# DRL-Navigation/DDRL4NAV

Hardware: AMD Instinct MI355X
Metric: env-steps/sec (whole node) + PPO update ms, Pong 256 envs at 1/2/4/8 GPUs (higher is better)
Workload: dtype f32 (f16x3 MFMA planes, fp32 accumulate)

## Files before the change

ddrl4nav_amd/csrc/fc2.hip:

```cpp
#include "engine2.h"

namespace ddrl {



struct FcFwdB {
  static constexpr int PITCH = 80, PLANE = 128 * PITCH, B_OFF = NPL * PLANE, LDS_BYTES = 2 * NPL * PLANE;
};

template <bool SPLIT>
__global__ __launch_bounds__(256) void fc_fwd_planes_kernel(const float* __restrict__ a3, int64_t a3_es, const unsigned short* __restrict__ wlb,
                                                            const float* __restrict__ amax, const float* __restrict__ params, int64_t bias_off0,
                                                            int64_t bias_off1, float* __restrict__ h, int64_t h_es, int n, int ne, int nsplit,
                                                            float* __restrict__ part, const float* __restrict__ smax, int smax_es) {
  using K = FcFwdB;
  extern __shared__ __attribute__((aligned(16))) char ldsf[];
  const int tid = threadIdx.x, lane = tid & 63, wave = tid >> 6, l31 = lane & 31, hi = lane >> 5;
  const int wr = wave >> 1, wc = wave & 1;
  int bx = blockIdx.x, by = blockIdx.y, bz = blockIdx.z;
  if (!SPLIT && (gridDim.y & 7) == 0) {
    const int lin = bx + 4 * by, xcd = lin & 7, q = lin >> 3;
    bx = q & 3, by = (q >> 2) * 8 + xcd;
  }
  if (SPLIT) {
    const int G = 4 * (int)gridDim.y, nz = (int)gridDim.z, lin = bx + 4 * by + G * bz, full = (nz & ~7) * G;
    int g, m;
    if (lin < full) {
      const int xcd = lin & 7, r = lin >> 3;
      g = (r / G) * 8 + xcd, m = r % G;
    } else {
      const int l2 = lin - full, xcd = l2 & 7, rest = nz & 7;
      if (rest == 4) {
        g = (nz & ~7) + (xcd >> 1), m = (l2 >> 3) * 2 + (xcd & 1);
      } else {
        g = (nz & ~7) + l2 / G, m = l2 % G;
      }
    }
    bz = g, bx = m & 3, by = m >> 2;
  }
  const int e = SPLIT ? bz % ne : bz, split = SPLIT ? bz / ne : 0, n0 = bx * 128, b0 = by * 128;
  float sa = plane_scale(amax[amax_idx(AMAX_A3, e)]), inv = 1.0f / (sa * plane_scale(amax[amax_idx(AMAX_WL, e)]));
  const int k4 = tid & 7, rr = tid >> 3;
  const float* asrc[4];
#pragma unroll
  for (int j = 0; j < 4; ++j) asrc[j] = a3 + e * a3_es + (int64_t)min(b0 + rr + 32 * j, n - 1) * FLAT + k4 * 4;
  const int k8 = tid & 3, cc = tid >> 2;
  const unsigned short* wsrc = wlb + (int64_t)e * 3 * FLAT * FEAT + (int64_t)(n0 + cc) * FLAT + k8 * 8;
  int aA[2], bB[2];
#pragma unroll
  for (int i = 0; i < 2; ++i) aA[i] = (wr * 64 + i * 32 + l31) * K::PITCH + hi * 16;
#pragma unroll
  for (int j = 0; j < 2; ++j) bB[j] = K::B_OFF + (wc * 64 + j * 32 + l31) * K::PITCH + hi * 16;
  constexpr int DEPTH = SPLIT ? 4 : 1;
  f4 ar[DEPTH][4], wrg[DEPTH][2][NPL];
  auto fetch = [&](int kb, int slot) {
#pragma unroll
    for (int j = 0; j < 4; ++j) ar[slot][j] = ld4(asrc[j] + kb * 32);
#pragma unroll
    for (int j = 0; j < 2; ++j)
#pragma unroll
      for (int p = 0; p < NPL; ++p) wrg[slot][j][p] = *(const f4*)(wsrc + (int64_t)p * FLAT * FEAT + (int64_t)j * 64 * FLAT + kb * 32);
  };
  auto commit = [&](int slot) {
#pragma unroll
    for (int j = 0; j < 4; ++j) {
      const f4 v = ar[slot][j];
      unsigned pa[NPL], pb[NPL];
      split_planes_c(v.x, v.y, sa, pa);
      split_planes_c(v.z, v.w, sa, pb);
      char* d = ldsf + (rr + 32 * j) * K::PITCH + k4 * 8;
#pragma unroll
      for (int p = 0; p < NPL; ++p) *(uint2*)(d + p * K::PLANE) = make_uint2(pa[p], pb[p]);
    }
#pragma unroll
    for (int j = 0; j < 2; ++j)
#pragma unroll
      for (int p = 0; p < NPL; ++p) *(f4*)(ldsf + K::B_OFF + p * K::PLANE + (cc + 64 * j) * K::PITCH + k8 * 16) = wrg[slot][j][p];
  };
  f32x16 acc[2][2];
#pragma unroll
  for (int i = 0; i < 2; ++i)
#pragma unroll
    for (int j = 0; j < 2; ++j)
#pragma unroll
      for (int r = 0; r < 16; ++r) acc[i][j][r] = 0.0f;
  auto compute = [&]() {
#pragma unroll
    for (int kg = 0; kg < 2; ++kg) {
      frag8 a[NPL][2], b[NPL][2];
#pragma unroll
      for (int p = 0; p < NPL; ++p) {
#pragma unroll
        for (int i = 0; i < 2; ++i) a[p][i] = *(const frag8*)(ldsf + aA[i] + p * K::PLANE + kg * 32);
#pragma unroll
        for (int j = 0; j < 2; ++j) b[p][j] = *(const frag8*)(ldsf + bB[j] + p * K::PLANE + kg * 32);
      }
#pragma unroll
      for (int t = 0; t < NPROD; ++t)
#pragma unroll
        for (int i = 0; i < 2; ++i)
#pragma unroll
          for (int j = 0; j < 2; ++j) acc[i][j] = mfma_planes(a[PA[t]][i], b[PB[t]][j], acc[i][j]);
    }
  };
  if constexpr (SPLIT) {
    constexpr int PER = (FLAT / 32) / FC_ACT_SPLITS;
    const int kb0 = split * PER;
#pragma unroll
    for (int d = 0; d < DEPTH && d < PER; ++d) fetch(kb0 + d, d);
    if (smax != nullptr) {
      float m = 0.0f;
      for (int i = tid; i < n; i += 256) m = fmaxf(m, smax[e * smax_es + i]);
      m = wave_fmax(m);
      float* red = (float*)ldsf;
      if (lane == 0) red[wave] = m;
      __syncthreads();
      const float a3top = fmaxf(fmaxf(red[0], red[1]), fmaxf(red[2], red[3]));
      __syncthreads();
      sa = plane_scale(a3top), inv = 1.0f / (sa * plane_scale(amax[amax_idx(AMAX_WL, e)]));
    }
    commit(0);
    if (DEPTH < PER) fetch(kb0 + DEPTH, 0);
    __syncthreads();
#pragma unroll
    for (int k = 0; k < PER; ++k) {
      compute();
      __syncthreads();
      if (k + 1 < PER) {
        commit((k + 1) % DEPTH);
        if (k + 1 + DEPTH < PER) fetch(kb0 + k + 1 + DEPTH, (k + 1) % DEPTH);
      }
      __syncthreads();
    }
  } else {
    constexpr int NKB = FLAT / 32;
    fetch(0, 0);
    commit(0);
    fetch(1, 0);
    __syncthreads();
    for (int kb = 0; kb < NKB; ++kb) {
      compute();
      __syncthreads();
      if (kb + 1 < NKB) {
        commit(0);
        if (kb + 2 < NKB) fetch(kb + 2, 0);
      }
      __syncthreads();
    }
  }
#pragma unroll
  for (int j = 0; j < 2; ++j) {
    const int nn = n0 + wc * 64 + j * 32 + l31;
    const float bias = SPLIT ? 0.0f : params[(e ? bias_off1 : bias_off0) + nn];
    float* dst = SPLIT ? part + ((int64_t)split * 2 + e) * n * FEAT : h + e * h_es;
#pragma unroll
    for (int i = 0; i < 2; ++i)
#pragma unroll
      for (int r = 0; r < 16; ++r) {
        const int b = b0 + wr * 64 + i * 32 + acc_row(r, hi);
        if (b < n) dst[(int64_t)b * FEAT + nn] = acc[i][j][r] * inv + bias;
      }
  }
}

void launch_fc_forward2(const EncCall& c, bool allow_split, hipStream_t st, bool per_sample_max) {
  const Workspace& w = *c.ws;
  const int64_t MB = c.max_batch;
  const int nsplit = allow_split ? fc_forward_splits(c.n) : 1;
  ProfRange pr(c.prof, nsplit > 1 ? "FcFwdSplit" : "FcFwd", st);
  {
    lds_limit_once<fc_fwd_planes_kernel<false>>((int)FcFwdB::LDS_BYTES);
    lds_limit_once<fc_fwd_planes_kernel<true>>((int)FcFwdB::LDS_BYTES);
    const dim3 grid(FEAT / 128, (c.n + 127) / 128, c.L->NE * nsplit);
    if (nsplit > 1)
      hipLaunchKernelGGL(fc_fwd_planes_kernel<true>, grid, dim3(256), FcFwdB::LDS_BYTES, st, w.a3, MB * FLAT, w.wlb, w.amax, c.params,
                         c.L->enc_base[0] + c.L->enc.lb, c.L->enc_base[c.L->NE - 1] + c.L->enc.lb, w.h, MB * FEAT, c.n, c.L->NE, nsplit, w.wpart,
                         per_sample_max ? w.actmax : (const float*)nullptr, ACT_FUSED_MAX);
    else
      hipLaunchKernelGGL(fc_fwd_planes_kernel<false>, grid, dim3(256), FcFwdB::LDS_BYTES, st, w.a3, MB * FLAT, w.wlb, w.amax, c.params,
                         c.L->enc_base[0] + c.L->enc.lb, c.L->enc_base[c.L->NE - 1] + c.L->enc.lb, w.h, MB * FEAT, c.n, c.L->NE, 1, w.wpart,
                         (const float*)nullptr, 0);
  }
}

struct FcDgradB {
  static constexpr int KBK = 32, WPE = 2, PITCH = 2 * KBK + 16, PLANE = 128 * PITCH, B_OFF = NPL * PLANE, LDS_BYTES = 2 * NPL * PLANE;
  static constexpr int NAQ = KBK / 4, ARJ = 128 * NAQ / 256, AROWS = 256 / NAQ;
  static constexpr int NWF = KBK / 8, WJ = 128 * NWF / 256, WCOLS = 256 / NWF;
};
__global__ __launch_bounds__(256) __attribute__((amdgpu_waves_per_eu(FcDgradB::WPE, FcDgradB::WPE))) void fc_dgrad_planes_kernel(const float* __restrict__ dh, int64_t dh_es, const unsigned short* __restrict__ wdlb,
                                                              float* __restrict__ amax, const unsigned* __restrict__ m3, float* __restrict__ dz3, int64_t a3_es, int n) {
  using K = FcDgradB;
  extern __shared__ __attribute__((aligned(16))) char ldsg[];
  const int tid = threadIdx.x, lane = tid & 63, wave = tid >> 6, l31 = lane & 31, hi = lane >> 5;
  const int wr = wave >> 1, wc = wave & 1;
  int bx = blockIdx.x, by = blockIdx.y;
  if ((gridDim.y & 7) == 0) {
    const int lin = bx + 25 * by, xcd = lin & 7, q = lin >> 3;
    if ((gridDim.y & 63) != 0) {
      bx = q % 25, by = (q / 25) * 8 + xcd;
    } else {
      const int blk = q / 40, r = q % 40;
      bx = (blk % 5) * 5 + r % 5, by = ((blk / 5) * 8 + r / 5) * 8 + xcd;
    }
  }
  const int e = blockIdx.z, k0 = bx * 128, b0 = by * 128;
  const float sa = plane_scale(amax[amax_idx(AMAX_DH, e)]), inv = 1.0f / (sa * plane_scale(amax[amax_idx(AMAX_WL, e)]));
  const int n4 = tid % K::NAQ, rr = tid / K::NAQ;
  const float* asrc[K::ARJ];
#pragma unroll
  for (int j = 0; j < K::ARJ; ++j) asrc[j] = dh + e * dh_es + (int64_t)min(b0 + rr + K::AROWS * j, n - 1) * FEAT + n4 * 4;
  const int n8 = tid % K::NWF, cc = tid / K::NWF;
  const unsigned short* wsrc[K::WJ];
#pragma unroll
  for (int j = 0; j < K::WJ; ++j) wsrc[j] = wdlb + (int64_t)e * 3 * FLAT * FEAT + (int64_t)min(k0 + cc + K::WCOLS * j, FLAT - 1) * FEAT + n8 * 8;
  int aA[2], bB[2];
#pragma unroll
  for (int i = 0; i < 2; ++i) aA[i] = (wr * 64 + i * 32 + l31) * K::PITCH + hi * 16;
#pragma unroll
  for (int j = 0; j < 2; ++j) bB[j] = K::B_OFF + (wc * 64 + j * 32 + l31) * K::PITCH + hi * 16;
  f4 ar[K::ARJ], wrg[K::WJ][NPL];
  auto fetch = [&](int kb) {
#pragma unroll
    for (int j = 0; j < K::ARJ; ++j) ar[j] = ld4(asrc[j] + kb * K::KBK);
#pragma unroll
    for (int j = 0; j < K::WJ; ++j)
#pragma unroll
      for (int p = 0; p < NPL; ++p) wrg[j][p] = *(const f4*)(wsrc[j] + (int64_t)p * FLAT * FEAT + kb * K::KBK);
  };
  auto commit = [&]() {
#pragma unroll
    for (int j = 0; j < K::ARJ; ++j) {
      const f4 v = ar[j];
      unsigned pa[NPL], pb[NPL];
      split_planes_c(v.x, v.y, sa, pa);
      split_planes_c(v.z, v.w, sa, pb);
      char* d = ldsg + (rr + K::AROWS * j) * K::PITCH + n4 * 8;
#pragma unroll
      for (int p = 0; p < NPL; ++p) *(uint2*)(d + p * K::PLANE) = make_uint2(pa[p], pb[p]);
    }
#pragma unroll
    for (int j = 0; j < K::WJ; ++j)
#pragma unroll
      for (int p = 0; p < NPL; ++p) *(f4*)(ldsg + K::B_OFF + p * K::PLANE + (cc + K::WCOLS * j) * K::PITCH + n8 * 16) = wrg[j][p];
  };
  f32x16 acc[2][2];
#pragma unroll
  for (int i = 0; i < 2; ++i)
#pragma unroll
    for (int j = 0; j < 2; ++j)
#pragma unroll
      for (int r = 0; r < 16; ++r) acc[i][j][r] = 0.0f;
  constexpr int NKB = FEAT / K::KBK;
  fetch(0);
  commit();
  fetch(1);
  __syncthreads();
  for (int kb = 0; kb < NKB; ++kb) {
#pragma unroll
    for (int kg = 0; kg < K::KBK / 16; ++kg) {
      frag8 a[NPL][2], b[NPL][2];
#pragma unroll
      for (int p = 0; p < NPL; ++p) {
#pragma unroll
        for (int i = 0; i < 2; ++i) a[p][i] = *(const frag8*)(ldsg + aA[i] + p * K::PLANE + kg * 32);
#pragma unroll
        for (int j = 0; j < 2; ++j) b[p][j] = *(const frag8*)(ldsg + bB[j] + p * K::PLANE + kg * 32);
      }
#pragma unroll
      for (int t = 0; t < NPROD; ++t)
#pragma unroll
        for (int i = 0; i < 2; ++i)
#pragma unroll
          for (int j = 0; j < 2; ++j) acc[i][j] = mfma_planes(a[PA[t]][i], b[PB[t]][j], acc[i][j]);
    }
    __syncthreads();
    if (kb + 1 < NKB) {
      commit();
      if (kb + 2 < NKB) fetch(kb + 2);
    }
    __syncthreads();
  }
  float big = 0.0f;
#pragma unroll
  for (int j = 0; j < 2; ++j) {
    const int k = k0 + wc * 64 + j * 32 + l31;
    if (k >= FLAT) continue;
    const int ch = k / 49, pix = k % 49;
    const int mbit = 16 * (ch >> 5) + 15 - ((ch & 3) + 4 * ((ch & 31) >> 3));
    const unsigned* mp = m3 + (int64_t)e * (a3_es / FLAT) * 98 + pix * 2 + ((ch >> 2) & 1);
#pragma unroll
    for (int i = 0; i < 2; ++i) {
      unsigned mw[16];
#pragma unroll
      for (int r = 0; r < 16; ++r) {
        const int b = min(b0 + wr * 64 + i * 32 + acc_row(r, hi), n - 1);
        mw[r] = mp[(int64_t)b * 98];
      }
#pragma unroll
      for (int r = 0; r < 16; ++r) {
        const int b = b0 + wr * 64 + i * 32 + acc_row(r, hi);
        const float g = leaky_bit(mw[r], mbit, acc[i][j][r] * inv);
        if (b < n) {
          dz3[e * a3_es + (int64_t)b * FLAT + k] = g;
          big = fmaxf(big, fabsf(g));
        }
      }
    }
  }
  amax_update(big, amax + amax_idx(AMAX_DZ3, e));
}

struct FcWgradB {
  static constexpr int KB = 32, PITCH = 320, PLANE = KB * PITCH, B_OFF = NPL * PLANE, LDS_BYTES = 2 * NPL * PLANE;
  static constexpr int64_t SLAB = (int64_t)FEAT * FLAT + FEAT;
};

__global__ __launch_bounds__(256) void fc_wgrad_planes_kernel(const float* __restrict__ dh, int64_t dh_es, const float* __restrict__ a3,
                                                              int64_t a3_es, const float* __restrict__ amax, const float* __restrict__ gsc,
                                                              int64_t gsc_es, float* __restrict__ part, int n, int nsplit, int ne) {
  using K = FcWgradB;
  extern __shared__ __attribute__((aligned(16))) char ldsw[];
  const int tid = threadIdx.x, lane = tid & 63, wave = tid >> 6, l31 = lane & 31, hi = lane >> 5;
  const int wr = wave >> 1, wc = wave & 1;
  const int unit = (int)(blockIdx.x >> 5) * 8 + (int)(blockIdx.x & 7);
  if (unit >= 25 * ne * nsplit) return;
  const int bx = unit % 25, by = (int)(blockIdx.x >> 3) & 3, bz = unit / 25;
  const int e = bz % ne, split = bz / ne;
  const float sd = WGRAD_HEADROOM * plane_scale(amax[amax_idx(AMAX_DH, e)]) / amax[amax_idx(AMAX_GMAX, e)], sa = plane_scale(amax[amax_idx(AMAX_A3, e)]),
              inv = 1.0f / (sd * sa);
  const float* gs = gsc + e * gsc_es;
  const int k0 = bx * 128, n0 = by * 128;
  const int nkb = (n + K::KB - 1) / K::KB;
  const int per = (nkb + nsplit - 1) / nsplit;
  const int kb_begin = split * per, kb_end = min(nkb, kb_begin + per);
  const int c4 = tid & 31, kk = tid >> 5;
  const float* dsrc = dh + e * dh_es + n0 + c4 * 4;
  const float* asrc = a3 + e * a3_es + min(k0 + c4 * 4, FLAT - 4);
  const int g16 = lane >> 4, q = (lane >> 2) & 3, pp = lane & 3;
  int aA[2], bB[2];
#pragma unroll
  for (int i = 0; i < 2; ++i) aA[i] = (8 * (g16 >> 1) + q) * K::PITCH + (wr * 64 + i * 32 + 16 * (g16 & 1) + 4 * pp) * 2;
#pragma unroll
  for (int j = 0; j < 2; ++j) bB[j] = K::B_OFF + (8 * (g16 >> 1) + q) * K::PITCH + (wc * 64 + j * 32 + 16 * (g16 & 1) + 4 * pp) * 2;
  f4 dr[4], ar[4];
  float gr[4];
  f4 bsum = zero4();
  const bool bias_owner = (bx == 0);
  auto fetch = [&](int kb) {
#pragma unroll
    for (int j = 0; j < 4; ++j) {
      const int64_t row = min(kb * K::KB + kk + 8 * j, n - 1);
      dr[j] = ld4(dsrc + row * FEAT);
      ar[j] = ld4(asrc + row * FLAT);
      gr[j] = gs[row];
    }
  };
  auto commit = [&](int kb) {
    if (kb * K::KB + K::KB > n) {
      rare_path();
#pragma unroll
      for (int j = 0; j < 4; ++j)
        if (kb * K::KB + kk + 8 * j >= n) dr[j] = zero4();
      rare_path();
    }
#pragma unroll
    for (int j = 0; j < 4; ++j) {
      char* d = ldsw + (kk + 8 * j) * K::PITCH + c4 * 8;
      unsigned pa[NPL], pb[NPL];
      const float sdj = sd * gr[j];
      split_planes(dr[j].x, dr[j].y, sdj, pa);
      split_planes(dr[j].z, dr[j].w, sdj, pb);
#pragma unroll
      for (int p = 0; p < NPL; ++p) *(uint2*)(d + p * K::PLANE) = make_uint2(pa[p], pb[p]);
      split_planes(ar[j].x, ar[j].y, sa, pa);
      split_planes(ar[j].z, ar[j].w, sa, pb);
#pragma unroll
      for (int p = 0; p < NPL; ++p) *(uint2*)(d + K::B_OFF + p * K::PLANE) = make_uint2(pa[p], pb[p]);
    }
    if (bias_owner) bsum += (dr[0] * gr[0] + dr[1] * gr[1]) + (dr[2] * gr[2] + dr[3] * gr[3]);
  };
  f32x16 acc[2][2];
#pragma unroll
  for (int i = 0; i < 2; ++i)
#pragma unroll
    for (int j = 0; j < 2; ++j)
#pragma unroll
      for (int r = 0; r < 16; ++r) acc[i][j][r] = 0.0f;
  if (kb_begin < kb_end) {
    fetch(kb_begin);
    commit(kb_begin);
    if (kb_begin + 1 < kb_end) fetch(kb_begin + 1);
    __syncthreads();
    for (int kb = kb_begin; kb < kb_end; ++kb) {
#pragma unroll
      for (int kg = 0; kg < 2; ++kg) {
        frag8 a[NPL][2], b[NPL][2];
#pragma unroll
        for (int p = 0; p < NPL; ++p) {
          const int off = p * K::PLANE + kg * 16 * K::PITCH;
#pragma unroll
          for (int i = 0; i < 2; ++i) a[p][i] = tr_frag(ldsw, aA[i] + off, aA[i] + off + 4 * K::PITCH);
#pragma unroll
          for (int j = 0; j < 2; ++j) b[p][j] = tr_frag(ldsw, bB[j] + off, bB[j] + off + 4 * K::PITCH);
        }
#pragma unroll
        for (int t = 0; t < NPROD; ++t)
#pragma unroll
          for (int i = 0; i < 2; ++i)
#pragma unroll
            for (int j = 0; j < 2; ++j) acc[i][j] = mfma_planes(a[PA[t]][i], b[PB[t]][j], acc[i][j]);
      }
      __syncthreads();
      if (kb + 1 < kb_end) {
        commit(kb + 1);
        if (kb + 2 < kb_end) fetch(kb + 2);
      }
      __syncthreads();
    }
  }
  float* slab = part + ((int64_t)split * 2 + e) * K::SLAB;
#pragma unroll
  for (int j = 0; j < 2; ++j) {
    const int k = k0 + wc * 64 + j * 32 + l31;
    if (k >= FLAT) continue;
#pragma unroll
    for (int i = 0; i < 2; ++i)
#pragma unroll
      for (int r = 0; r < 16; ++r) slab[(int64_t)(n0 + wr * 64 + i * 32 + acc_row(r, hi)) * FLAT + k] = acc[i][j][r] * inv;
  }
  if (bias_owner) {
    float* red = (float*)ldsw;
    st4(red + kk * 128 + c4 * 4, bsum);
    __syncthreads();
    if (tid < 128) {
      float s = 0.0f;
#pragma unroll
      for (int t = 0; t < 8; ++t) s += red[t * 128 + tid];
      slab[(int64_t)FEAT * FLAT + n0 + tid] = s;
    }
  }
}

void launch_fc_backward2(const EncCall& c, float* grads, hipStream_t st, int part) {
  const Workspace& w = *c.ws;
  const int64_t MB = c.max_batch;
  const ParamLayout& L = *c.L;
  const int S = c.splits->fc;
  if (part != 1) {
    {
      ProfRange pr(c.prof, "FcWgrad", st);
      lds_limit_once<fc_wgrad_planes_kernel>((int)FcWgradB::LDS_BYTES);
      const dim3 wgrid((unsigned)((25 * L.NE * S + 7) / 8 * 32));
      hipLaunchKernelGGL(fc_wgrad_planes_kernel, wgrid, dim3(256), FcWgradB::LDS_BYTES, st, w.dh, MB * FEAT, w.a3, MB * FLAT, w.amax, w.gsc, MB,
                         w.wpart, c.n, S, L.NE);
    }
    ProfRange pr(c.prof, "reduce_partials", st);
    launch_reduce_partials(w.wpart, S, FcWgradB::SLAB, L.NE, grads, L.enc_base[0] + L.enc.lw, L.enc_base[1] + L.enc.lw, st);
  }
  if (part != 2) {
    ProfRange pr(c.prof, "FcDgrad", st);
    lds_limit_once<fc_dgrad_planes_kernel>((int)FcDgradB::LDS_BYTES);
    hipLaunchKernelGGL(fc_dgrad_planes_kernel, dim3((FLAT + 127) / 128, (c.n + 127) / 128, L.NE), dim3(256), FcDgradB::LDS_BYTES, st, w.dh, MB * FEAT,
                       w.wdlb, w.amax, w.m3, w.dz3, MB * FLAT, c.n);
  }
}

}
```

Measured before the change: 262,200.

## Retile FC dgrad kernel to 128x224 tiles with exact column coverage

Reshapes the FC data-gradient GEMM tile from 128x128 (2x2 waves, each 64x64) to 128 rows by 224 columns, where each wave owns 32 rows and all 7 column fragments. Since 224 divides FLAT (3136) exactly, the padded, clamped last column tile and its wasted MFMA work go away, and each wave reuses its A fragment across 7 B fragments. The XCD block swizzle is reworked for 14 column tiles. In exchange, LDS and accumulator register use per block grow and the grid has fewer blocks, which may reduce occupancy or cause spills at WPE=2.

```diff
diff --git a/ddrl4nav_amd/csrc/fc2.hip b/ddrl4nav_amd/csrc/fc2.hip
--- a/ddrl4nav_amd/csrc/fc2.hip
+++ b/ddrl4nav_amd/csrc/fc2.hip
@@ -184,49 +184,47 @@
 }
 
 struct FcDgradB {
-  static constexpr int KBK = 32, WPE = 2, PITCH = 2 * KBK + 16, PLANE = 128 * PITCH, B_OFF = NPL * PLANE, LDS_BYTES = 2 * NPL * PLANE;
-  static constexpr int NAQ = KBK / 4, ARJ = 128 * NAQ / 256, AROWS = 256 / NAQ;
-  static constexpr int NWF = KBK / 8, WJ = 128 * NWF / 256, WCOLS = 256 / NWF;
+  static constexpr int KBK = 32, WPE = 2, NW = 4, THREADS = 64 * NW, TM = 32 * NW, TN = 224, NF = TN / 32, NCT = FLAT / TN, PITCH = 2 * KBK + 16;
+  static constexpr int PLANE_A = TM * PITCH, PLANE_B = TN * PITCH, B_OFF = NPL * PLANE_A, LDS_BYTES = NPL * (PLANE_A + PLANE_B);
+  static constexpr int NAQ = KBK / 4, ARJ = TM * NAQ / THREADS, AROWS = THREADS / NAQ;
+  static constexpr int NWF = KBK / 8, WCOLS = THREADS / NWF, WJ = (TN + WCOLS - 1) / WCOLS;
+  static_assert(NCT * TN == FLAT && NF * 32 == TN, "the column tiles cover the matrix without padding");
 };
-__global__ __launch_bounds__(256) __attribute__((amdgpu_waves_per_eu(FcDgradB::WPE, FcDgradB::WPE))) void fc_dgrad_planes_kernel(const float* __restrict__ dh, int64_t dh_es, const unsigned short* __restrict__ wdlb,
+__global__ __launch_bounds__(FcDgradB::THREADS) __attribute__((amdgpu_waves_per_eu(FcDgradB::WPE, FcDgradB::WPE))) void fc_dgrad_planes_kernel(const float* __restrict__ dh, int64_t dh_es, const unsigned short* __restrict__ wdlb,
                                                               float* __restrict__ amax, const unsigned* __restrict__ m3, float* __restrict__ dz3, int64_t a3_es, int n) {
   using K = FcDgradB;
   extern __shared__ __attribute__((aligned(16))) char ldsg[];
   const int tid = threadIdx.x, lane = tid & 63, wave = tid >> 6, l31 = lane & 31, hi = lane >> 5;
-  const int wr = wave >> 1, wc = wave & 1;
   int bx = blockIdx.x, by = blockIdx.y;
   if ((gridDim.y & 7) == 0) {
-    const int lin = bx + 25 * by, xcd = lin & 7, q = lin >> 3;
+    const int lin = bx + K::NCT * by, xcd = lin & 7, q = lin >> 3;
     if ((gridDim.y & 63) != 0) {
-      bx = q % 25, by = (q / 25) * 8 + xcd;
+      bx = q % K::NCT, by = (q / K::NCT) * 8 + xcd;
     } else {
-      const int blk = q / 40, r = q % 40;
-      bx = (blk % 5) * 5 + r % 5, by = ((blk / 5) * 8 + r / 5) * 8 + xcd;
-    }
-  }
-  const int e = blockIdx.z, k0 = bx * 128, b0 = by * 128;
+      const int blk = q / 56, r = q % 56;
+      bx = (blk % 2) * 7 + r % 7, by = ((blk / 2) * 8 + r / 7) * 8 + xcd;
+    }
+  }
+  const int e = blockIdx.z, k0 = bx * K::TN, b0 = by * K::TM;
   const float sa = plane_scale(amax[amax_idx(AMAX_DH, e)]), inv = 1.0f / (sa * plane_scale(amax[amax_idx(AMAX_WL, e)]));
   const int n4 = tid % K::NAQ, rr = tid / K::NAQ;
   const float* asrc[K::ARJ];
 #pragma unroll
   for (int j = 0; j < K::ARJ; ++j) asrc[j] = dh + e * dh_es + (int64_t)min(b0 + rr + K::AROWS * j, n - 1) * FEAT + n4 * 4;
   const int n8 = tid % K::NWF, cc = tid / K::NWF;
-  const unsigned short* wsrc[K::WJ];
-#pragma unroll
-  for (int j = 0; j < K::WJ; ++j) wsrc[j] = wdlb + (int64_t)e * 3 * FLAT * FEAT + (int64_t)min(k0 + cc + K::WCOLS * j, FLAT - 1) * FEAT + n8 * 8;
-  int aA[2], bB[2];
-#pragma unroll
-  for (int i = 0; i < 2; ++i) aA[i] = (wr * 64 + i * 32 + l31) * K::PITCH + hi * 16;
-#pragma unroll
-  for (int j = 0; j < 2; ++j) bB[j] = K::B_OFF + (wc * 64 + j * 32 + l31) * K::PITCH + hi * 16;
+  const unsigned short* wsrc = wdlb + (int64_t)e * 3 * FLAT * FEAT + (int64_t)(k0 + cc) * FEAT + n8 * 8;
+  const bool wlast = cc + K::WCOLS * (K::WJ - 1) < K::TN;
+  const int aA = (wave * 32 + l31) * K::PITCH + hi * 16, bB = K::B_OFF + l31 * K::PITCH + hi * 16;
   f4 ar[K::ARJ], wrg[K::WJ][NPL];
   auto fetch = [&](int kb) {
 #pragma unroll
     for (int j = 0; j < K::ARJ; ++j) ar[j] = ld4(asrc[j] + kb * K::KBK);
 #pragma unroll
-    for (int j = 0; j < K::WJ; ++j)
-#pragma unroll
-      for (int p = 0; p < NPL; ++p) wrg[j][p] = *(const f4*)(wsrc[j] + (int64_t)p * FLAT * FEAT + kb * K::KBK);
+    for (int j = 0; j < K::WJ; ++j) {
+      if (j == K::WJ - 1 && !wlast) break;
+#pragma unroll
+      for (int p = 0; p < NPL; ++p) wrg[j][p] = *(const f4*)(wsrc + (int64_t)p * FLAT * FEAT + (int64_t)j * K::WCOLS * FEAT + kb * K::KBK);
+    }
   };
   auto commit = [&]() {
 #pragma unroll
@@ -237,20 +235,20 @@
       split_planes_c(v.z, v.w, sa, pb);
       char* d = ldsg + (rr + K::AROWS * j) * K::PITCH + n4 * 8;
 #pragma unroll
-      for (int p = 0; p < NPL; ++p) *(uint2*)(d + p * K::PLANE) = make_uint2(pa[p], pb[p]);
-    }
-#pragma unroll
-    for (int j = 0; j < K::WJ; ++j)
-#pragma unroll
-      for (int p = 0; p < NPL; ++p) *(f4*)(ldsg + K::B_OFF + p * K::PLANE + (cc + K::WCOLS * j) * K::PITCH + n8 * 16) = wrg[j][p];
-  };
-  f32x16 acc[2][2];
-#pragma unroll
-  for (int i = 0; i < 2; ++i)
-#pragma unroll
-    for (int j = 0; j < 2; ++j)
-#pragma unroll
-      for (int r = 0; r < 16; ++r) acc[i][j][r] = 0.0f;
+      for (int p = 0; p < NPL; ++p) *(uint2*)(d + p * K::PLANE_A) = make_uint2(pa[p], pb[p]);
+    }
+#pragma unroll
+    for (int j = 0; j < K::WJ; ++j) {
+      if (j == K::WJ - 1 && !wlast) break;
+#pragma unroll
+      for (int p = 0; p < NPL; ++p) *(f4*)(ldsg + K::B_OFF + p * K::PLANE_B + (cc + K::WCOLS * j) * K::PITCH + n8 * 16) = wrg[j][p];
+    }
+  };
+  f32x16 acc[K::NF];
+#pragma unroll
+  for (int j = 0; j < K::NF; ++j)
+#pragma unroll
+    for (int r = 0; r < 16; ++r) acc[j][r] = 0.0f;
   constexpr int NKB = FEAT / K::KBK;
   fetch(0);
   commit();
@@ -259,20 +257,17 @@
   for (int kb = 0; kb < NKB; ++kb) {
 #pragma unroll
     for (int kg = 0; kg < K::KBK / 16; ++kg) {
-      frag8 a[NPL][2], b[NPL][2];
+      frag8 a[NPL], b[NPL][K::NF];
 #pragma unroll
       for (int p = 0; p < NPL; ++p) {
-#pragma unroll
-        for (int i = 0; i < 2; ++i) a[p][i] = *(const frag8*)(ldsg + aA[i] + p * K::PLANE + kg * 32);
-#pragma unroll
-        for (int j = 0; j < 2; ++j) b[p][j] = *(const frag8*)(ldsg + bB[j] + p * K::PLANE + kg * 32);
+        a[p] = *(const frag8*)(ldsg + aA + p * K::PLANE_A + kg * 32);
+#pragma unroll
+        for (int j = 0; j < K::NF; ++j) b[p][j] = *(const frag8*)(ldsg + bB + j * 32 * K::PITCH + p * K::PLANE_B + kg * 32);
       }
 #pragma unroll
       for (int t = 0; t < NPROD; ++t)
 #pragma unroll
-        for (int i = 0; i < 2; ++i)
-#pragma unroll
-          for (int j = 0; j < 2; ++j) acc[i][j] = mfma_planes(a[PA[t]][i], b[PB[t]][j], acc[i][j]);
+        for (int j = 0; j < K::NF; ++j) acc[j] = mfma_planes(a[PA[t]], b[PB[t]][j], acc[j]);
     }
     __syncthreads();
     if (kb + 1 < NKB) {
@@ -283,28 +278,24 @@
   }
   float big = 0.0f;
 #pragma unroll
-  for (int j = 0; j < 2; ++j) {
-    const int k = k0 + wc * 64 + j * 32 + l31;
-    if (k >= FLAT) continue;
+  for (int j = 0; j < K::NF; ++j) {
+    const int k = k0 + j * 32 + l31;
     const int ch = k / 49, pix = k % 49;
     const int mbit = 16 * (ch >> 5) + 15 - ((ch & 3) + 4 * ((ch & 31) >> 3));
     const unsigned* mp = m3 + (int64_t)e * (a3_es / FLAT) * 98 + pix * 2 + ((ch >> 2) & 1);
-#pragma unroll
-    for (int i = 0; i < 2; ++i) {
-      unsigned mw[16];
-#pragma unroll
-      for (int r = 0; r < 16; ++r) {
-        const int b = min(b0 + wr * 64 + i * 32 + acc_row(r, hi), n - 1);
-        mw[r] = mp[(int64_t)b * 98];
-      }
-#pragma unroll
-      for (int r = 0; r < 16; ++r) {
-        const int b = b0 + wr * 64 + i * 32 + acc_row(r, hi);
-        const float g = leaky_bit(mw[r], mbit, acc[i][j][r] * inv);
-        if (b < n) {
-          dz3[e * a3_es + (int64_t)b * FLAT + k] = g;
-          big = fmaxf(big, fabsf(g));
-        }
+    unsigned mw[16];
+#pragma unroll
+    for (int r = 0; r < 16; ++r) {
+      const int b = min(b0 + wave * 32 + acc_row(r, hi), n - 1);
+      mw[r] = mp[(int64_t)b * 98];
+    }
+#pragma unroll
+    for (int r = 0; r < 16; ++r) {
+      const int b = b0 + wave * 32 + acc_row(r, hi);
+      const float g = leaky_bit(mw[r], mbit, acc[j][r] * inv);
+      if (b < n) {
+        dz3[e * a3_es + (int64_t)b * FLAT + k] = g;
+        big = fmaxf(big, fabsf(g));
       }
     }
   }
@@ -460,8 +451,9 @@
   }
   if (part != 2) {
     ProfRange pr(c.prof, "FcDgrad", st);
-    lds_limit_once<fc_dgrad_planes_kernel>((int)FcDgradB::LDS_BYTES);
-    hipLaunchKernelGGL(fc_dgrad_planes_kernel, dim3((FLAT + 127) / 128, (c.n + 127) / 128, L.NE), dim3(256), FcDgradB::LDS_BYTES, st, w.dh, MB * FEAT,
+    using K = FcDgradB;
+    lds_limit_once<fc_dgrad_planes_kernel>((int)K::LDS_BYTES);
+    hipLaunchKernelGGL(fc_dgrad_planes_kernel, dim3(K::NCT, (c.n + K::TM - 1) / K::TM, L.NE), dim3(K::THREADS), K::LDS_BYTES, st, w.dh, MB * FEAT,
                        w.wdlb, w.amax, w.m3, w.dz3, MB * FLAT, c.n);
   }
 }
```

Result: no change. 262,300, median of 5 (+0.0%).
